# reazon-research/ReazonSpeech

Hardware: AMD Instinct MI355X
Metric: RTFx (audio-sec/wall-sec), FastConformer-RNNT 619M batch=256 (higher is better)
Workload: dtype bf16

## Files before the change

reazonspeech_amd/csrc/k_conformer.hip:

```cpp
#include <algorithm>

#include "rs_common.h"

extern "C" int rs_create(rs_ctx** out, int device, const rs_dims* dims) {
    if (!out || !dims) return RS_EINVAL;
    *out = nullptr;
    rs_ctx* ctx = new (std::nothrow) rs_ctx();
    rs_conformer* state = ctx ? new (std::nothrow) rs_conformer() : nullptr;
    if (!state) { delete ctx; return RS_EINVAL; }
    rs_conformer& cf = *state;
    ctx->family = RS_FAM_CONFORMER;
    ctx->state.reset(state);
    ctx->device = device;
    ctx->d = *dims;
    const rs_dims& d = ctx->d;
    int rc = RS_OK;
    if (d.n_heads <= 0 || d.d_model % d.n_heads || (d.d_model / d.n_heads != 128 && d.d_model / d.n_heads != 64))
        rc = rs_fail(ctx, RS_EINVAL, "head_dim must be 128 or 64 (d_model %d, heads %d)", d.d_model, d.n_heads);
    else if (d.d_model % 256 || d.ff_dim % 64) rc = rs_fail(ctx, RS_EINVAL, "d_model %% 256, ff_dim %% 64 required");
    else if (d.sub_stages < 2 || d.sub_stages > 4) rc = rs_fail(ctx, RS_EINVAL, "2..4 subsampling stages supported");
    else if (d.n_layers < 1) rc = rs_fail(ctx, RS_EINVAL, "n_layers");
    else if (d.pred_layers < 1 || d.pred_layers > 4) rc = rs_fail(ctx, RS_EINVAL, "pred_layers");
    else if ((unsigned)d.frontend_kind > 1u  || (unsigned)d.sub_kind > 1u || (unsigned)d.final_norm > 1u || (unsigned)d.joint_act > 1u)
        rc = rs_fail(ctx, RS_EINVAL, "model family switches must be 0 or 1");
// ... 295 lines not shown
        RS_TRY(gemm(ctxb, dm, L32.pw2_w, dm, x, dm, M, dm, RES, L.pw2_b, 1.0f, x));
        RS_TRY(rs_launch_layernorm(ctx, x, L.ln_ff2_g, L.ln_ff2_b, M, dm, d.ln_eps, nullptr, hn, s));
        RS_TRY(gemm(hn, dm, L32.ff2_w1, dm, big, ff, M, ff, RS_GEMM_BIAS | RS_GEMM_SILU, L.ff2_b1, 1.0f, nullptr));
        RS_TRY(gemm(big, ff, L32.ff2_w2, ff, x, dm, M, dm, RES, L.ff2_b2, 0.5f, x));
        RS_TRY(rs_launch_layernorm(ctx, x, L.ln_out_g, L.ln_out_b, M, dm, d.ln_eps, nullptr, x, s));
        for (size_t k = 0; k < cf.tap_ids.size(); ++k)
            if (cf.tap_ids[k] == i)
                RS_HIP(ctx, hipMemcpyAsync(cf.tap_layers + k * (size_t)M * dm, x, (size_t)M * dm * 4, hipMemcpyDeviceToDevice, s));
    }
    if (d.final_norm) RS_TRY(rs_launch_layernorm(ctx, x, cf.final_norm_g, cf.final_norm_b, M, dm, d.ln_eps, nullptr, x, s));
    if (enc_out) RS_HIP(ctx, hipMemcpyAsync(enc_out, x, (size_t)M * dm * 4, hipMemcpyDeviceToDevice, s));
    RS_TRY(gemm(x, dm, w.jenc_w, dm, joint_enc, d.joint_hidden, M, d.joint_hidden, RS_GEMM_BIAS, ctx->jenc_b, 1.0f, nullptr));
    if (d.ctc_vocab > 0 && (cf.ctc_probs || cf.ctc_blank)) {
        const int Vp = rs_ctc_pad(d.ctc_vocab);
        float* z = cf.ctc_probs ? cf.ctc_probs : pl.ctc;
        RS_TRY(gemm(x, dm, w.ctc_w, dm, z, Vp, M, Vp, RS_GEMM_BIAS, cf.ctc_b, 1.0f, nullptr));
        RS_TRY(rs_launch_ctc_softmax(ctx, z, M, d.ctc_vocab, Vp, d.blank_id, cf.ctc_blank, s));
    }
#undef RS_TRY
    return RS_OK;
}

}

size_t rs_conformer_workspace_bytes_impl(const rs_ctx* ctx, int B, int t_max) {
    rs_arena measure;
    plan_encoder(ctx, B, t_max > 0 ? t_max : 1, measure);
    size_t enc = measure.bytes() + ENC_SLACK;
    if (ctx->has_f32) {
        const size_t enc32 = encoder_f32_workspace_bytes(ctx, B, t_max > 0 ? t_max : 1);
        if (enc32 > enc) enc = enc32;
    }
    return enc;
}

int rs_conformer_encoder_forward_impl(rs_ctx* ctx, const float* feats, const int32_t* n_frames, int B, int t_max, float* enc_out, float* joint_enc,
                                      int32_t* enc_lens, void* workspace, size_t workspace_bytes, hipStream_t s) {
    if (ctx->precision_f32)
        return rs_encoder_forward_f32(ctx, feats, n_frames, B, t_max, enc_out, joint_enc, enc_lens, workspace, workspace_bytes, s);
    const rs_dims& d = ctx->d;
    const rs_conformer& cf = *rs_conformer_of(ctx);
    rs_arena arena(workspace);
    const EncPlan pl = plan_encoder(ctx, B, t_max, arena);
    if (workspace_bytes < arena.bytes() + ENC_SLACK)
        return rs_fail(ctx, RS_EWORKSPACE, "encoder: workspace %zu < %zu", workspace_bytes, arena.bytes() + ENC_SLACK);
    int32_t* const lens_stage = pl.lens;
    uint16_t *const sa = pl.sa, *const sb = pl.sb, *const hn = pl.hn, *const big = pl.big, *const ctxb = pl.ctxb, *const posp = pl.posp;
    float *const x = pl.x, *const ln_stats = pl.stats;
    const int C = d.sub_channels, dm = d.d_model, ff = d.ff_dim, S = d.sub_stages;
    const int Tp = pl.T[S], M = B * Tp;
    int rc;
#define RS_TRY(call) do { rc = (call); if (rc != RS_OK) return rc; } while (0)

    RS_TRY(rs_launch_enc_lens(ctx, n_frames, B, lens_stage, s));
    if (Tp <= 0) return rs_fail(ctx, RS_EINVAL, "encoder: %d feature frames are too few for the subsampling", t_max);
    if (d.sub_kind == 1) {
        uint16_t* const col = pl.col;
        const int T1 = pl.T[1], F1 = pl.F[1], T2 = pl.T[2], F2 = pl.F[2];
        for (int b0 = 0; b0 < B; b0 += pl.chunk) {
            const int bc = B - b0 < pl.chunk ? B - b0 : pl.chunk;
            RS_TRY(rs_launch_sub2d_conv0(ctx, feats, lens_stage, b0, bc, t_max, T1, F1, sa, s));
            const bool patches_in_place = col == nullptr;
            if (!patches_in_place) RS_TRY(rs_launch_im2col3x3s2(ctx, sa, bc, T1, F1, T2, F2, col, s));
            rs_gemm_args g{};
            if (patches_in_place) { g.A = sa; g.conv_C = C; g.conv_T1 = T1; g.conv_F1 = F1; g.conv_T2 = T2; g.conv_F2 = F2; }
            else g.A = col;
            g.lda = 9 * C; g.W = cf.sub_conv1_w; g.ldw = 9 * C; g.out = sb + (size_t)b0 * T2 * F2 * C; g.ldc = C;
            g.M = bc * T2 * F2; g.N = C; g.K = 9 * C;
            g.flags = RS_GEMM_BIAS | RS_GEMM_RELU | RS_GEMM_ROWMASK; g.bias = cf.sub_conv1_b; g.alpha = 1.0f;
            g.mask_lens = lens_stage + B + b0; g.mask_rows_per_step = F2; g.mask_steps = T2;
            RS_TRY(rs_launch_gemm(ctx, g, s));
        }
    } else
    RS_TRY(rs_launch_sub_conv0_dw1(ctx, feats, lens_stage, B, t_max, pl.T[2], pl.F[2], sa, s));
    for (int st = 2; st <= S && d.sub_kind == 0; ++st) {
        if (st > 2)
            RS_TRY(rs_launch_sub_dw(ctx, sb, cf.sub_dw_w[st - 2], cf.sub_dw_b[st - 2], lens_stage + (st - 1) * B, st, B,
                                    pl.T[st - 1], pl.F[st - 1], pl.T[st], pl.F[st], sa, s));
        rs_gemm_args g{};
        g.A = sa; g.lda = C; g.W = cf.sub_pw_w[st - 2]; g.ldw = C; g.out = sb; g.ldc = C;
        g.M = B * pl.T[st] * pl.F[st]; g.N = C; g.K = C;
        g.flags = RS_GEMM_BIAS | RS_GEMM_RELU | RS_GEMM_ROWMASK; g.bias = cf.sub_pw_b[st - 2]; g.alpha = 1.0f;
        g.mask_lens = lens_stage + (st - 1) * B; g.mask_rows_per_step = pl.F[st]; g.mask_steps = pl.T[st];
        RS_TRY(rs_launch_gemm(ctx, g, s));
    }
    {
        rs_gemm_args g{};
        const int K = C * pl.F[S];
        g.A = sb; g.lda = K; g.W = cf.sub_out_w; g.ldw = K; g.out = x; g.ldc = dm; g.M = M; g.N = dm; g.K = K;
        g.flags = RS_GEMM_BIAS | RS_GEMM_OUT_F32; g.bias = cf.sub_out_b;
        g.alpha = d.xscaling ? sqrtf((float)dm) : 1.0f;
        RS_TRY(rs_launch_gemm(ctx, g, s));
    }
    const int32_t* lens = lens_stage + (S - 1) * B;
    RS_HIP(ctx, hipMemcpyAsync(enc_lens, lens, (size_t)B * 4, hipMemcpyDeviceToDevice, s));
    if (cf.tap_sub) RS_HIP(ctx, hipMemcpyAsync(cf.tap_sub, x, (size_t)M * dm * 4, hipMemcpyDeviceToDevice, s));

    const int tcap = (int)((cf.pos_table_bytes / ((size_t)dm * 2) + 1) / 2);
    if (Tp > tcap) return rs_fail(ctx, RS_EINVAL, "encoder: T'=%d exceeds the registered pos.table capacity %d", Tp, tcap);
    const uint16_t* pos_slice = cf.pos_table + (size_t)(tcap - Tp) * dm;
    const int npos = 2 * Tp - 1;

    const rs_layer_w* res_ln = nullptr;
    auto gemm = [&](const uint16_t* A, int lda, const uint16_t* W, int K, void* out, int ldc, int Mr, int N, int flags,
                    const float* bias, float alpha, const float* res) -> int {
        rs_gemm_args g{};
        g.A = A; g.lda = lda; g.W = W; g.ldw = K; g.out = out; g.ldc = ldc; g.M = Mr; g.N = N; g.K = K;
        g.flags = flags; g.bias = bias; g.alpha = alpha; g.residual = res;
        if (res && res_ln) { g.res_ln_stats = ln_stats; g.res_ln_g = res_ln->ln_out_g; g.res_ln_b = res_ln->ln_out_b; res_ln = nullptr; }
        return rs_launch_gemm(ctx, g, s);
    };
    const int RES = RS_GEMM_BIAS | RS_GEMM_RESIDUAL | RS_GEMM_OUT_F32;
    const bool glu_fused = cf.fuse_glu != 0 && (dm % 32) == 0;

    for (int i = 0; i < d.n_layers; ++i) {
        const rs_layer_w& L = cf.layers[i];
        const bool last = i == d.n_layers - 1;
        if (i == 0) RS_TRY(rs_launch_layernorm(ctx, x, L.ln_ff1_g, L.ln_ff1_b, M, dm, d.ln_eps, hn, nullptr, s));
        RS_TRY(gemm(hn, dm, L.ff1_w1, dm, big, ff, M, ff, RS_GEMM_BIAS | RS_GEMM_SILU, L.ff1_b1, 1.0f, nullptr));
        RS_TRY(gemm(big, ff, L.ff1_w2, ff, x, dm, M, dm, RES, L.ff1_b2, 0.5f, x));
        RS_TRY(rs_launch_layernorm(ctx, x, L.ln_att_g, L.ln_att_b, M, dm, d.ln_eps, hn, nullptr, s));
        RS_TRY(gemm(hn, dm, L.qkv_w, dm, big, 3 * dm, M, 3 * dm, RS_GEMM_BIAS, L.qkv_b, 1.0f, nullptr));
        const uint16_t* pproj = posp;
        if (L.pos_proj) pproj = L.pos_proj + (size_t)(tcap - Tp) * dm;
        else RS_TRY(gemm(pos_slice, dm, L.pos_w, dm, posp, dm, npos, dm, 0, nullptr, 1.0f, nullptr));
        RS_TRY(rs_launch_attention(ctx, big, pproj, L.bias_u, L.bias_v, lens, B, Tp, ctxb, s));
        RS_TRY(gemm(ctxb, dm, L.out_w, dm, x, dm, M, dm, RES, L.out_b, 1.0f, x));
        RS_TRY(rs_launch_layernorm(ctx, x, L.ln_conv_g, L.ln_conv_b, M, dm, d.ln_eps, hn, nullptr, s));
        if (glu_fused) {
            RS_TRY(gemm(hn, dm, L.pw1_w, dm, big, dm, M, 2 * dm, RS_GEMM_BIAS | RS_GEMM_GLU, L.pw1_b, 1.0f, nullptr));
            RS_TRY(rs_launch_glu_dwconv(ctx, big, RS_GLU_APPLIED, L.dw_w, L.dw_b, lens, B, Tp, dm, d.conv_kernel, ctxb, s));
        } else {
            RS_TRY(gemm(hn, dm, L.pw1_w, dm, big, 2 * dm, M, 2 * dm, RS_GEMM_BIAS, L.pw1_b, 1.0f, nullptr));
            RS_TRY(rs_launch_glu_dwconv(ctx, big, RS_GLU_BLOCK32, L.dw_w, L.dw_b, lens, B, Tp, dm, d.conv_kernel, ctxb, s));
        }
        RS_TRY(gemm(ctxb, dm, L.pw2_w, dm, x, dm, M, dm, RES, L.pw2_b, 1.0f, x));
        RS_TRY(rs_launch_layernorm(ctx, x, L.ln_ff2_g, L.ln_ff2_b, M, dm, d.ln_eps, hn, nullptr, s));
        RS_TRY(gemm(hn, dm, L.ff2_w1, dm, big, ff, M, ff, RS_GEMM_BIAS | RS_GEMM_SILU, L.ff2_b1, 1.0f, nullptr));
        RS_TRY(gemm(big, ff, L.ff2_w2, ff, x, dm, M, dm, RES, L.ff2_b2, 0.5f, x));
        if (last && d.final_norm) {
            RS_TRY(rs_launch_layernorm(ctx, x, L.ln_out_g, L.ln_out_b, M, dm, d.ln_eps, nullptr, x, s));
        } else if (last) {
            bool want_f32 = enc_out != nullptr;
            for (size_t k = 0; k < cf.tap_ids.size(); ++k) want_f32 = want_f32 || cf.tap_ids[k] == i;
            RS_TRY(rs_launch_layernorm(ctx, x, L.ln_out_g, L.ln_out_b, M, dm, d.ln_eps, hn, want_f32 ? x : nullptr, s));
        } else {
            const rs_layer_w& Ln = cf.layers[i + 1];
            bool tapped = cf.defer_out_norm == 0;
            for (size_t k = 0; k < cf.tap_ids.size(); ++k) tapped = tapped || cf.tap_ids[k] == i;
            RS_TRY(rs_launch_layernorm2(ctx, x, L.ln_out_g, L.ln_out_b, Ln.ln_ff1_g, Ln.ln_ff1_b, M, dm, d.ln_eps,
                                        tapped ? x : nullptr, hn, tapped ? nullptr : ln_stats, s));
            if (!tapped) res_ln = &L;
        }
        for (size_t k = 0; k < cf.tap_ids.size(); ++k)
            if (cf.tap_ids[k] == i)
                RS_HIP(ctx, hipMemcpyAsync(cf.tap_layers + k * (size_t)M * dm, x, (size_t)M * dm * 4, hipMemcpyDeviceToDevice, s));
    }
    if (d.final_norm) RS_TRY(rs_launch_layernorm(ctx, x, cf.final_norm_g, cf.final_norm_b, M, dm, d.ln_eps, hn, enc_out ? x : nullptr, s));
    if (enc_out) RS_HIP(ctx, hipMemcpyAsync(enc_out, x, (size_t)M * dm * 4, hipMemcpyDeviceToDevice, s));
    RS_TRY(gemm(hn, dm, ctx->jenc_w, dm, joint_enc, d.joint_hidden, M, d.joint_hidden, RS_GEMM_BIAS | RS_GEMM_OUT_F32,
                ctx->jenc_b, 1.0f, nullptr));
    if (d.ctc_vocab > 0 && (cf.ctc_probs || cf.ctc_blank)) {
        float* z = cf.ctc_probs ? cf.ctc_probs : pl.ctc;
        const int Vp = rs_ctc_pad(d.ctc_vocab);
        RS_TRY(gemm(hn, dm, cf.ctc_w, dm, z, Vp, M, Vp, RS_GEMM_BIAS | RS_GEMM_OUT_F32, cf.ctc_b, 1.0f, nullptr));
        RS_TRY(rs_launch_ctc_softmax(ctx, z, M, d.ctc_vocab, Vp, d.blank_id, cf.ctc_blank, s));
    }
// ... 4 lines not shown
```

reazonspeech_amd/csrc/k_subsample.hip:

```cpp
#include "rs_common.h"

namespace {

__global__ void enc_lens_kernel(const int32_t* __restrict__ n_frames, int B, int stages, int sub_kind, int32_t* __restrict__ out) {
    const int b = blockIdx.x * blockDim.x + threadIdx.x;
    if (b >= B) return;
    int n = n_frames[b];
    for (int s = 0; s < stages; ++s) {
        n = n > 0 ? (sub_kind ? (n >= 3 ? (n - 3) / 2 + 1 : 0) : (n + 2 - 3) / 2 + 1) : 0;
        out[s * B + b] = n;
    }
}

__device__ __forceinline__ void put(uint16_t* p, float v) { *p = f32_to_bf16(v); }
__device__ __forceinline__ void put(float* p, float v) { *p = v; }

template <typename OT>
__global__ __launch_bounds__(256) void sub_conv0_dw1_kernel(
    const float* __restrict__ feats, const int32_t* __restrict__ lens_stage , int B, int t_max,
    int n_mels, int T2, int F1, int F2, int C, const float* __restrict__ w0 ,
    const float* __restrict__ b0, const float* __restrict__ wd , const float* __restrict__ bd,
    OT* __restrict__ out) {
    const int b = blockIdx.y, t2 = blockIdx.x, c = threadIdx.x;
    const int L1 = lens_stage[0 * B + b], L2 = lens_stage[1 * B + b];
// ... 292 lines not shown
        float wt[9][8], bs[8];
#pragma unroll
        for (int k = 0; k < 9; ++k) {
            const float4 w0 = reinterpret_cast<const float4*>(w + k * C + c)[0], w1 = reinterpret_cast<const float4*>(w + k * C + c)[1];
            wt[k][0] = w0.x; wt[k][1] = w0.y; wt[k][2] = w0.z; wt[k][3] = w0.w; wt[k][4] = w1.x; wt[k][5] = w1.y; wt[k][6] = w1.z; wt[k][7] = w1.w;
        }
        {
            const float4 b0 = reinterpret_cast<const float4*>(bias + c)[0], b1 = reinterpret_cast<const float4*>(bias + c)[1];
            bs[0] = b0.x; bs[1] = b0.y; bs[2] = b0.z; bs[3] = b0.w; bs[4] = b1.x; bs[5] = b1.y; bs[6] = b1.z; bs[7] = b1.w;
        }
        bool jok[3];
#pragma unroll
        for (int j = 0; j < 3; ++j) { const int fi = 2 * fo - 1 + j; jok[j] = fi >= 0 && fi < Fin; }
        const uint16_t* ibase = in + ((size_t)b * Tin * Fin) * C + c;
        auto load_row = [&](int ti, u16x8_t (&x)[3]) {
#pragma unroll
            for (int j = 0; j < 3; ++j) {
                if (jok[j]) x[j] = *reinterpret_cast<const u16x8_t*>(ibase + ((size_t)ti * Fin + (2 * fo - 1 + j)) * C);
                else
#pragma unroll
                    for (int e = 0; e < 8; ++e) x[j][e] = 0;
            }
        };
        u16x8_t top[3], mid[3], bot[3];
#pragma unroll
        for (int j = 0; j < 3; ++j)
#pragma unroll
            for (int e = 0; e < 8; ++e) { top[j][e] = 0; mid[j][e] = 0; bot[j][e] = 0; }
        bool top_ok = to_first > 0 && 2 * to_first - 1 < Tin;
        if (top_ok) load_row(2 * to_first - 1, top);
        u16x8_t mid_next[3], bot_next[3];
#pragma unroll
        for (int j = 0; j < 3; ++j) { mid_next[j] = mid[j]; bot_next[j] = bot[j]; }
        if (2 * to_first < Tin) load_row(2 * to_first, mid_next);
        if (2 * to_first + 1 < Tin) load_row(2 * to_first + 1, bot_next);
        for (int to = to_first; to < to_live; ++to) {
            const bool mid_ok = 2 * to < Tin, bot_ok = 2 * to + 1 < Tin;
#pragma unroll
            for (int j = 0; j < 3; ++j) { mid[j] = mid_next[j]; bot[j] = bot_next[j]; }
            if (to + 1 < to_live) {
                if (2 * to + 2 < Tin) load_row(2 * to + 2, mid_next);
                if (2 * to + 3 < Tin) load_row(2 * to + 3, bot_next);
            }
            float acc[8];
#pragma unroll
            for (int e = 0; e < 8; ++e) acc[e] = bs[e];
            if (top_ok) dw_taps(acc, wt, 0, top, jok);
            if (mid_ok) dw_taps(acc, wt, 1, mid, jok);
            if (bot_ok) dw_taps(acc, wt, 2, bot, jok);
            u16x8_t o;
#pragma unroll
            for (int e = 0; e < 8; ++e) o[e] = f32_to_bf16(acc[e]);
            *reinterpret_cast<u16x8_t*>(obase + ((size_t)to * Fout) * C) = o;
#pragma unroll
            for (int j = 0; j < 3; ++j) top[j] = bot[j];
            top_ok = bot_ok;
        }
    }
    u16x8_t z;
#pragma unroll
    for (int e = 0; e < 8; ++e) z[e] = 0;
    for (int to = max(to_first, to_live); to < to_end; ++to) *reinterpret_cast<u16x8_t*>(obase + ((size_t)to * Fout) * C) = z;
}

__global__ __launch_bounds__(256) void sub_dw_f32_kernel(const float* __restrict__ in, const float* __restrict__ w ,
                                                         const float* __restrict__ bias, const int32_t* __restrict__ lens_out,
                                                         int Tin, int Fin, int Tout, int Fout, int C, float* __restrict__ out) {
    const int c = threadIdx.x, fo = blockIdx.x, to = blockIdx.y, b = blockIdx.z;
    float* op = out + (((size_t)b * Tout + to) * Fout + fo) * C + c;
    if (to >= lens_out[b]) { *op = 0.0f; return; }
    float acc = bias[c];
#pragma unroll
    for (int i = 0; i < 3; ++i) {
        const int ti = 2 * to - 1 + i;
        if (ti < 0 || ti >= Tin) continue;
#pragma unroll
        for (int j = 0; j < 3; ++j) {
            const int fi = 2 * fo - 1 + j;
            if (fi < 0 || fi >= Fin) continue;
            acc = fmaf(w[(i * 3 + j) * C + c], in[(((size_t)b * Tin + ti) * Fin + fi) * C + c], acc);
        }
    }
    *op = acc;
}

}

int rs_launch_enc_lens(rs_ctx* ctx, const int32_t* n_frames, int B, int32_t* lens_out, hipStream_t s) {
    hipLaunchKernelGGL(enc_lens_kernel, dim3((B + 127) / 128), dim3(128), 0, s, n_frames, B, ctx->d.sub_stages, ctx->d.sub_kind, lens_out);
    RS_CHECK_LAUNCH(ctx, "enc_lens");
    return RS_OK;
}

constexpr int SUB_F2 = 20;
static bool conv0_run_form(int F2) { return F2 == SUB_F2 && !rs_knob(RS_KNOB_SUB_CONV0_OLD); }

int rs_launch_sub_conv0_dw1(rs_ctx* ctx, const float* feats, const int32_t* lens_stage, int B, int t_max, int T2,
                            int F2, uint16_t* out, hipStream_t s) {
    const rs_dims& d = ctx->d;
    const rs_conformer& cf = *rs_conformer_of(ctx);
    const int C = d.sub_channels;
    if (C > 256 || (C % 64)) return rs_fail(ctx, RS_EINVAL, "subsampling: channels %d unsupported (<=256, %%64)", C);
    const int F1 = (d.n_mels + 2 - 3) / 2 + 1;
    if (d.n_mels % 4 || 4 * F2 > d.n_mels || 2 * F2 < F1)
        return rs_fail(ctx, RS_EINVAL, "subsampling: n_mels=%d must be a multiple of 4 with 4*F2 <= n_mels", d.n_mels);
    const size_t lds = 0;
    const double flops = (double)B * T2 * F2 * C * 2.0 * (6 * 9 + 9);
    const double bytes = (double)B * t_max * d.n_mels * 4.0 + (double)B * T2 * F2 * C * 2.0;
    rs_prof_scope prof(ctx, RS_PROF_SUBSAMPLE, s, flops, bytes);
    if (conv0_run_form(F2))
        hipLaunchKernelGGL((sub_conv0_dw1_run_kernel<uint16_t, SUB_F2>), dim3((T2 + SUB_RUN - 1) / SUB_RUN, B), dim3(C / 2), lds, s, feats,
                           lens_stage, B, t_max, d.n_mels, T2, C, cf.sub_conv0_w, cf.sub_conv0_b, cf.sub_dw_w[0], cf.sub_dw_b[0], out);
    else
        hipLaunchKernelGGL(sub_conv0_dw1_kernel<uint16_t>, dim3(T2, B), dim3(C), lds, s, feats, lens_stage, B, t_max, d.n_mels, T2,
                       F1, F2, C, cf.sub_conv0_w, cf.sub_conv0_b, cf.sub_dw_w[0], cf.sub_dw_b[0], out);
    prof.end();
    RS_CHECK_LAUNCH(ctx, "sub_conv0_dw1");
    return RS_OK;
}

int rs_launch_sub_dw(rs_ctx* ctx, const uint16_t* in, const float* w, const float* b, const int32_t* lens_out,
                     int stage, int B, int t_in, int f_in, int t_out, int f_out, uint16_t* out, hipStream_t s) {
    (void)stage;
    const int C = ctx->d.sub_channels;
    const int cgs = C / 8;
    const int fpb = 256 / cgs;
    const dim3 grid((f_out + fpb - 1) / fpb, t_out, B), block(cgs * fpb);
    const double bytes = (double)B * C * 2.0 * ((double)t_in * f_in + (double)t_out * f_out);
    rs_prof_scope prof(ctx, RS_PROF_SUBSAMPLE, s, (double)B * t_out * f_out * C * 18.0, bytes);
    if (!rs_knob(RS_KNOB_SUB_DW_OLD) && cgs * f_out <= 512)
        hipLaunchKernelGGL(sub_dw_run_kernel, dim3((t_out + DW_RUN - 1) / DW_RUN, B), dim3(cgs * f_out), 0, s, in, w, b, lens_out, t_in,
                           f_in, t_out, f_out, C, out);
    else
        hipLaunchKernelGGL(sub_dw_kernel, grid, block, 0, s, in, w, b, lens_out, t_in, f_in, t_out, f_out, C, out);
    prof.end();
    RS_CHECK_LAUNCH(ctx, "sub_dw");
    return RS_OK;
}

int rs_launch_sub_conv0_dw1_f32(rs_ctx* ctx, const float* feats, const int32_t* lens_stage, int B, int t_max, int T2, int F2,
                                float* out, hipStream_t s) {
    const rs_dims& d = ctx->d;
    const rs_conformer& cf = *rs_conformer_of(ctx);
    const int C = d.sub_channels;
    if (C > 256 || (C % 64)) return rs_fail(ctx, RS_EINVAL, "subsampling: channels %d unsupported (<=256, %%64)", C);
    const int F1 = (d.n_mels + 2 - 3) / 2 + 1;
    if (d.n_mels % 4 || 4 * F2 > d.n_mels || 2 * F2 < F1)
        return rs_fail(ctx, RS_EINVAL, "subsampling: n_mels=%d must be a multiple of 4 with 4*F2 <= n_mels", d.n_mels);
    rs_prof_scope prof(ctx, RS_PROF_SUBSAMPLE, s, (double)B * T2 * F2 * C * 2.0 * (6 * 9 + 9),
                       (double)B * t_max * d.n_mels * 4.0 + (double)B * T2 * F2 * C * 4.0);
    if (conv0_run_form(F2))
        hipLaunchKernelGGL((sub_conv0_dw1_run_kernel<float, SUB_F2>), dim3((T2 + SUB_RUN - 1) / SUB_RUN, B), dim3(C / 2), 0, s, feats,
                           lens_stage, B, t_max, d.n_mels, T2, C, cf.sub_conv0_w, cf.sub_conv0_b, cf.sub_dw_w[0], cf.sub_dw_b[0], out);
    else
        hipLaunchKernelGGL(sub_conv0_dw1_kernel<float>, dim3(T2, B), dim3(C), 0, s, feats, lens_stage, B, t_max, d.n_mels, T2, F1, F2, C,
                       cf.sub_conv0_w, cf.sub_conv0_b, cf.sub_dw_w[0], cf.sub_dw_b[0], out);
    prof.end();
    RS_CHECK_LAUNCH(ctx, "sub_conv0_dw1_f32");
    return RS_OK;
}

int rs_launch_sub_dw_f32(rs_ctx* ctx, const float* in, const float* w, const float* b, const int32_t* lens_out, int B, int t_in,
                         int f_in, int t_out, int f_out, float* out, hipStream_t s) {
    const int C = ctx->d.sub_channels;
    rs_prof_scope prof(ctx, RS_PROF_SUBSAMPLE, s, (double)B * t_out * f_out * C * 18.0,
                       (double)B * C * 4.0 * ((double)t_in * f_in + (double)t_out * f_out));
    hipLaunchKernelGGL(sub_dw_f32_kernel, dim3(f_out, t_out, B), dim3(C), 0, s, in, w, b, lens_out, t_in, f_in, t_out, f_out, C, out);
    prof.end();
    RS_CHECK_LAUNCH(ctx, "sub_dw_f32");
    return RS_OK;
}
```

reazonspeech_amd/csrc/rs_common.h:

```cpp
#pragma once
#include <hip/hip_runtime.h>
#include <stdint.h>
#include <stdio.h>
#include <memory>
#include <string>
#include <unordered_map>
#include <vector>

#include "../../include/rs_asr.h"
#include "rs_arena.h"
#include "rs_family.h"
#include "rs_knobs.h"
#include "rs_tensors.h"

typedef __bf16 bf16x8_t __attribute__((ext_vector_type(8)));
typedef float f32x4_t __attribute__((ext_vector_type(4)));
typedef float f32x16_t __attribute__((ext_vector_type(16)));
typedef unsigned short u16x8_t __attribute__((ext_vector_type(8)));
typedef unsigned short u16x4_t __attribute__((ext_vector_type(4)));

__device__ __forceinline__ float bf16_to_f32(unsigned short v) {
    return __uint_as_float(((unsigned)v) << 16);
}
typedef __bf16 bf16x4_t __attribute__((ext_vector_type(4)));
// ... 124 lines not shown
    void* wfm_scratch = nullptr;
    size_t wfm_scratch_bytes = 0;
    int prof_mask = 0;
    rs_prof_slot prof[8];
    int32_t prof_tag[4] = {0, 0, 0, 0};
};

inline rs_conformer* rs_conformer_of(const rs_ctx* ctx) {
    return ctx && ctx->family == RS_FAM_CONFORMER ? static_cast<rs_conformer*>(ctx->state.get()) : nullptr;
}
rs_k2* rs_k2_of(const rs_ctx* ctx);
rs_avsr* rs_avsr_of(const rs_ctx* ctx);

int rs_ensure_dynamic_lds(rs_ctx* ctx, const void* func, int bytes);

int rs_fail(rs_ctx* ctx, int code, const char* fmt, ...);

inline int rs_guard(rs_ctx* ctx, rs_entry e) {
    char msg[512];
    const int rc = rs_family_guard(e, ctx != nullptr, ctx ? ctx->family : RS_FAM_CONFORMER, ctx && ctx->finalized, msg, sizeof msg);
    if (rc != RS_OK && ctx) ctx->err = msg;
    return rc;
}
inline bool rs_guard_query(const rs_ctx* ctx, rs_entry e) {
    return rs_family_guard(e, ctx != nullptr, ctx ? ctx->family : RS_FAM_CONFORMER, ctx && ctx->finalized, nullptr, 0) == RS_OK;
}
#define RS_GUARD(ctx, entry) do { if (const int _g = rs_guard((ctx), RS_ENTRY_##entry); _g != RS_OK) return _g; } while (0)
#define RS_GUARD_QUERY(ctx, entry, zero) do { if (!rs_guard_query((ctx), RS_ENTRY_##entry)) return zero; } while (0)

struct rs_weights : rs_tensor_reader {
    explicit rs_weights(const rs_ctx* ctx) : rs_tensor_reader(ctx->tensors) {}
    template <typename T>
    void get(const std::string& name, size_t elems, const T*& out) {
        const void* p = out;
        get_bytes(name, elems * sizeof(T), p);
        out = static_cast<const T*>(p);
    }
    int fail(rs_ctx* ctx) const { return rs_fail(ctx, rc, "%s", msg.c_str()); }
};
void rs_get_screened_joint(rs_ctx* ctx, rs_weights& r);
int rs_n_cus(rs_ctx* ctx);

#define RS_HIP(ctx, call)                                                              \
    do {                                                                               \
        hipError_t _e = (call);                                                        \
        if (_e != hipSuccess)                                                          \
            return rs_fail((ctx), RS_EHIP, "%s:%d %s -> %s", __FILE__, __LINE__, #call, \
                           hipGetErrorString(_e));                                     \
    } while (0)

#define RS_CHECK_LAUNCH(ctx, what)                                                            \
    do {                                                                                      \
        hipError_t _e = hipGetLastError();                                                    \
        if (_e != hipSuccess)                                                                 \
            return rs_fail((ctx), RS_EHIP, "launch %s failed: %s", (what), hipGetErrorString(_e)); \
    } while (0)

int rs_prof_class_index(int klass);
void rs_prof_begin(rs_ctx* ctx, int klass, hipStream_t s, double flops, double bytes);
void rs_prof_end(rs_ctx* ctx, int klass, hipStream_t s);
struct rs_prof_scope {
    rs_prof_scope(rs_ctx* ctx, int klass, hipStream_t s, double flops, double bytes) : ctx(ctx), klass(klass), s(s) { rs_prof_begin(ctx, klass, s, flops, bytes); }
    rs_prof_scope(const rs_prof_scope&) = delete;
    rs_prof_scope& operator=(const rs_prof_scope&) = delete;
    ~rs_prof_scope() { end(); }
    void end() { if (open) rs_prof_end(ctx, klass, s); open = false; }
private:
    rs_ctx* ctx; int klass; hipStream_t s; bool open = true;
};

struct rs_gemm_args {
    const uint16_t* A; int lda;
    const uint16_t* W; int ldw;
    void* out; int ldc;
    int M, N, K, flags;
    const float* bias; float alpha;
    const float* residual;
    const int32_t* mask_lens; int mask_rows_per_step; int mask_steps;
    const float* res_ln_stats; const float* res_ln_g; const float* res_ln_b;
    uint16_t* out_bf16; int ld_bf16;
    int conv_C, conv_T1, conv_F1, conv_T2, conv_F2;
};
int rs_launch_gemm(rs_ctx* ctx, const rs_gemm_args& a, hipStream_t s);
int rs_launch_layernorm(rs_ctx* ctx, const float* x, const float* g, const float* b, int M, int d, float eps,
                        uint16_t* out_bf16, float* out_f32, hipStream_t s);
int rs_launch_layernorm2(rs_ctx* ctx, const float* x, const float* g1, const float* b1, const float* g2, const float* b2,
                         int M, int d, float eps, float* out_f32, uint16_t* out_bf16, float* stats, hipStream_t s);
int rs_launch_attention(rs_ctx* ctx, const uint16_t* qkv, const uint16_t* pos, const float* bias_u,
                        const float* bias_v, const int32_t* lens, int B, int T, uint16_t* out, hipStream_t s);
int rs_launch_glu_dwconv(rs_ctx* ctx, const uint16_t* x, int layout, const float* w, const float* b, const int32_t* lens,
                         int B, int T, int d, int k, uint16_t* out, hipStream_t s);
int rs_launch_frontend(rs_ctx* ctx, const float* audio, const int32_t* lens, int B, int audio_stride,
                       int pad_left, int pad_right, int t_max, float* feats, int32_t* n_frames, float* raw,
                       hipStream_t s);
int rs_launch_sub_conv0_dw1(rs_ctx* ctx, const float* feats, const int32_t* lens_stage, int B, int t_max, int T2,
                            int F2, uint16_t* out, hipStream_t s);
int rs_launch_sub_dw(rs_ctx* ctx, const uint16_t* in, const float* w, const float* b, const int32_t* lens_out,
                     int stage, int B, int t_in, int f_in, int t_out, int f_out, uint16_t* out, hipStream_t s);
int rs_launch_gemm_f32(rs_ctx* ctx, const float* A, int lda, const float* W, int ldw, float* out, int ldc, int M, int N, int K,
                       int flags, const float* bias, float alpha, const float* residual, const int32_t* mask_lens,
                       int mask_rows_per_step, int mask_steps, hipStream_t s);
int rs_launch_conv3x3_f32(rs_ctx* ctx, const float* in, int n_img, int H, int Wd, int C, int OH, int OW, int stride, const float* W, int Cout,
                          const float* bn_scale, const float* bn_shift, const float* residual, const float* prelu, float* out, int one_by_one, hipStream_t s);
int rs_launch_gemm_f32_skinny(rs_ctx* ctx, const float* A, int lda, const float* W, int ldw, float* out, int ldc, int M, int N, int K, int flags,
                              const float* bias, const float* residual, hipStream_t s);
int rs_launch_attention_f32(rs_ctx* ctx, const float* qkv, const float* pos, const float* bias_u, const float* bias_v,
                            const int32_t* lens, int B, int T, float* out, hipStream_t s);
int rs_launch_glu_dwconv_f32(rs_ctx* ctx, const float* x, const float* w, const float* b, const int32_t* lens, int B, int T,
                             int d, int k, float* out, hipStream_t s);
int rs_launch_i8_range(rs_ctx* ctx, const float* A, int lda, const int32_t* lens, int group, int n_groups, int K, float* qp, hipStream_t s);
int rs_launch_gemm_i8q(rs_ctx* ctx, const float* A, int lda, int group, const float* qp, const int8_t* W, int ldw, const int32_t* colsum,
                       const float* wq, float* out, int ldc, int M, int N, int K, int flags, const float* bias, const float* residual, hipStream_t s);
int rs_launch_sub_conv0_dw1_f32(rs_ctx* ctx, const float* feats, const int32_t* lens_stage, int B, int t_max, int T2, int F2,
                                float* out, hipStream_t s);
int rs_launch_sub_dw_f32(rs_ctx* ctx, const float* in, const float* w, const float* b, const int32_t* lens_out, int B, int t_in,
                         int f_in, int t_out, int f_out, float* out, hipStream_t s);
int rs_launch_enc_lens(rs_ctx* ctx, const int32_t* n_frames, int B, int32_t* lens_out, hipStream_t s);
int rs_launch_sub2d_conv0(rs_ctx* ctx, const float* feats, const int32_t* lens1, int b0, int Bc, int t_max, int T1, int F1,
                          uint16_t* out, hipStream_t s);
int rs_launch_im2col3x3s2(rs_ctx* ctx, const uint16_t* in, int Bc, int T1, int F1, int T2, int F2, uint16_t* out, hipStream_t s);
int rs_launch_ctc_softmax(rs_ctx* ctx, float* logits, int M, int V, int ld, int blank, float* blank_out, hipStream_t s);
int rs_launch_sub2d_conv0_f32(rs_ctx* ctx, const float* feats, const int32_t* lens1, int b0, int Bc, int t_max, int T1, int F1,
                              float* out, hipStream_t s);
int rs_launch_im2col3x3s2_f32(rs_ctx* ctx, const float* in, int Bc, int T1, int F1, int T2, int F2, float* out, hipStream_t s);
static inline int rs_ctc_pad(int v) { return (v + 3) / 4 * 4; }
int rs_conformer_finalize_impl(rs_ctx* ctx);
size_t rs_conformer_workspace_bytes_impl(const rs_ctx* ctx, int B, int t_max);
int rs_conformer_encoder_forward_impl(rs_ctx* ctx, const float* feats, const int32_t* n_frames, int B, int t_max, float* enc_out, float* joint_enc,
                                      int32_t* enc_lens, void* workspace, size_t workspace_bytes, hipStream_t s);
int rs_avsr_finalize_impl(rs_ctx* ctx);
const rs_avsr_dims* rs_avsr_dims_of(const rs_ctx* ctx);
int rs_k2_finalize_impl(rs_ctx* ctx);
int rs_k2_unk_id(const rs_ctx* ctx);
size_t rs_k2_workspace_bytes_impl(const rs_ctx* ctx, int B, int t_max);
int rs_k2_enc_frames_impl(const rs_ctx* ctx, int n_feat);
int rs_k2_encoder_forward_impl(rs_ctx* ctx, const float* feats, const int32_t* n_frames, int B, int t_max, float* enc_out, float* joint_enc,
                               int32_t* enc_lens, void* workspace, size_t workspace_bytes, hipStream_t s);
int rs_launch_dwconv_act(rs_ctx* ctx, const uint16_t* x, const float* w, const float* b, const int32_t* lens, int B, int T, int d, int k,
                         int act, uint16_t* out, hipStream_t s);
static inline int rs_conv_len(int n, int sub_kind) { return sub_kind ? (n >= 3 ? (n - 3) / 2 + 1 : 0) : (n > 0 ? (n + 2 - 3) / 2 + 1 : 0); }
```

reazonspeech_amd/csrc/rs_knobs.h:

```cpp
#pragma once
#include <stdlib.h>
#include <string.h>

#include <atomic>
#include <mutex>

#include "../../include/rs_asr.h"

#define RS_KNOBS(X)                                                                                                                   \
    X(GEMM_TILE, "RS_GEMM_TILE", INT, 0, "forced GEMM tile height (256 / 192 / 128 / 64); 0 = by shape")                              \
    X(GEMM_GROUP_M, "RS_GEMM_GROUP_M", INT, 0, "row panels per XCD tile group; 0 = by shape")                                         \
    X(GEMM_PAIRS, "RS_GEMM_PAIRS", INT, 2, "2 = two tiles per workgroup, LDS ring carried over; 1 = ring restarted; 0 = one tile")    \
    X(GEMM_BREG, "RS_GEMM_BREG", INT, 0, "1 = 256- / 192-row launches keep the weight operand out of LDS (global -> VGPR)")           \
    X(ATTN_PERSIST, "RS_ATTN_PERSIST", INT, 0, "1 = full attention on resident workgroups that walk the items (n >= 2: on n)")        \
    X(ATTN_STREAM, "RS_ATTN_STREAM", INT, 0, "1 = the streaming attention form (+ 16 x mask: phases left out, for timing)")           \
    X(ATTN64, "RS_ATTN64", INT, 4, "head_dim 64: key blocks per chunk; 0 = the one-workgroup-per-CU geometry")                        \
    X(ATTN64_NW, "RS_ATTN64_NW", INT, 4, "head_dim 64: waves per workgroup (the second number of $RS_ATTN64)")                        \
    X(ATTN_F32_OLD, "RS_ATTN_F32_OLD", PRESENT, 0, "float32 attention: the first form (one wave per key sum)")                        \
    X(ATTN_F32_KEYS, "RS_ATTN_F32_KEYS", PRESENT, 0, "float32 attention: the second form (keys over lanes, no MFMA)")                 \
    X(GLU_GENERIC, "RS_GLU_GENERIC", INT, 0, "GLU + depthwise conv: 1 = the any-kernel-size path, 2 = the f32-tile kernel on the gated layout") \
    X(SUB_IM2COL, "RS_SUB_IM2COL", PRESENT, 0, "ESPnet subsampling: gather the 3 x 3 patches into a matrix first (sizes the workspace too)") \
    X(FUSE_GLU, "RS_FUSE_GLU", INT, 1, "context default: 0 = GLU in the depthwise kernel, not the pw1 GEMM epilogue")                 \
    X(DEFER_OUT_NORM, "RS_DEFER_OUT_NORM", INT, 1, "context default: 0 = every output norm stores its f32 rows")                      \
    X(DECODE_SCREEN, "RS_DECODE_SCREEN", INT, 1, "context default: 0 = exact evaluation of every joint column")                       \
    X(DECODE_NARROW, "RS_DECODE_NARROW", INT, 1, "context default: 0 = the wide-tile LSTM / projection kernels")                      \
    X(DECODE_NO_XCD, "RS_DECODE_NO_XCD", PRESENT, 0, "greedy decode: joint grids not padded to a multiple of 8 column tiles")         \
    X(DECODE_NO_LOOKAHEAD, "RS_DECODE_NO_LOOKAHEAD", PRESENT, 0, "greedy decode: one frame per utterance and step at every batch size") \
    X(VERIFY_WIDE, "RS_VERIFY_WIDE", INT, 0, "screened joint: 1 = a workgroup per row for V <= 3072 too")                             \
    X(DECODE_TRACE, "RS_DECODE_TRACE", PRESENT, 0, "greedy decode: print the step count of every call to stderr")                     \
    X(BEAM_SPEC, "RS_BEAM_SPEC", INT, 3, "beam search: evaluations asked for per iteration (1 .. 8; sizes the workspace too)")         \
    X(BEAM_TRACE, "RS_BEAM_TRACE", PRESENT, 0, "beam search: phase timing of the step kernel")                                        \
    X(BEAM_RECORD_LDS, "RS_BEAM_RECORD_LDS", PRESENT, 0, "beam search: the any-vocabulary record kernel on a small vocabulary")       \
    X(LOGMEL_OLD, "RS_LOGMEL_OLD", PRESENT, 0, "log-mel: the first form (16 frames per workgroup, filterbank read from global memory)") \
    X(SUB_CONV0_OLD, "RS_SUB_CONV0_OLD", PRESENT, 0, "conv0 + dw1: the first form (a workgroup per output row, every odd conv0 row twice)") \
    X(SUB_DW_OLD, "RS_SUB_DW_OLD", PRESENT, 0, "bf16 depthwise stage: the first form (a thread per output bin, every input row read by two rows)") \
    X(AVSR_POSCONV_OLD, "RS_AVSR_POSCONV_OLD", PRESENT, 0, "AV-HuBERT positional convolution: the VALU form")                         \
    X(K2_CONV1_OLD, "RS_K2_CONV1_OLD", PRESENT, 0, "Zipformer conv1: the VALU form (the one other channel counts run)")               \
    X(K2_ATTW_SWEEPS, "RS_K2_ATTW_SWEEPS", INT, 1, "Zipformer attention weights: 3 = the three-sweep kernel")                         \
    X(K2_CONV2_FUSED, "RS_K2_CONV2_FUSED", INT, 1, "default of option k2_conv2_fused: 0 = patch matrix + GEMM launch")                \
    X(K2_CNX_FUSED, "RS_K2_CNX_FUSED", INT, 1, "default of option k2_cnx_fused: 0 = the ConvNeXt pointwise pair as two GEMM launches")

enum rs_knob_id {
#define RS_KNOB_ENUM(id, env, kind, def, what) RS_KNOB_##id,
    RS_KNOBS(RS_KNOB_ENUM)
#undef RS_KNOB_ENUM
    RS_KNOB_COUNT
};
enum rs_knob_kind { RS_KNOB_PRESENT, RS_KNOB_INT };
struct rs_knob_row { const char* env; rs_knob_kind kind; int def; };
static const rs_knob_row rs_knob_rows[RS_KNOB_COUNT] = {
#define RS_KNOB_ROW(id, env, kind, def, what) {env, RS_KNOB_##kind, def},
    RS_KNOBS(RS_KNOB_ROW)
#undef RS_KNOB_ROW
};

struct rs_knob_table {
    std::atomic<int> value[RS_KNOB_COUNT];
    std::atomic<bool> given[RS_KNOB_COUNT];
    std::once_flag once;
};
inline rs_knob_table rs_knob_state;

inline void rs_knobs_read_env() {
    std::call_once(rs_knob_state.once, [] {
        rs_knob_table& t = rs_knob_state;
        for (int i = 0; i < RS_KNOB_COUNT; ++i) { t.value[i] = rs_knob_rows[i].def; t.given[i] = false; }
        for (int i = 0; i < RS_KNOB_COUNT; ++i) {
            const char* e = i == RS_KNOB_ATTN64_NW ? nullptr : getenv(rs_knob_rows[i].env);
            if (!e) continue;
            t.given[i] = true;
            t.value[i] = rs_knob_rows[i].kind == RS_KNOB_PRESENT ? 1 : atoi(e);
            if (i == RS_KNOB_ATTN64) {
                t.given[RS_KNOB_ATTN64_NW] = true;
                if (const char* c = strchr(e, ',')) t.value[RS_KNOB_ATTN64_NW] = atoi(c + 1);
            }
        }
    });
}

inline int rs_knob(rs_knob_id id) { rs_knobs_read_env(); return rs_knob_state.value[id].load(std::memory_order_relaxed); }
inline bool rs_knob_given(rs_knob_id id) { rs_knobs_read_env(); return rs_knob_state.given[id].load(std::memory_order_relaxed); }
inline void rs_knob_set(rs_knob_id id, int v) { rs_knobs_read_env(); rs_knob_state.value[id].store(v, std::memory_order_relaxed); }

inline int rs_knob_find(const char* env_name) {
    for (int i = 0; env_name && i < RS_KNOB_COUNT; ++i)
        if (!strcmp(env_name, rs_knob_rows[i].env)) return i;
    return -1;
}
inline int rs_knob_set_named(const char* env_name, int v) {
    const int i = rs_knob_find(env_name);
    if (i < 0) return RS_EINVAL;
    rs_knob_set((rs_knob_id)i, v);
    return RS_OK;
}
inline int rs_knob_get_named(const char* env_name, int* v) {
    const int i = rs_knob_find(env_name);
    if (i < 0 || !v) return RS_EINVAL;
    *v = rs_knob((rs_knob_id)i);
    return RS_OK;
}
```

Before: 47280.

## Add persistent streaming MFMA kernel for 256-channel subsampling pointwise convs

Routes the 256x256 pointwise convolutions of the subsampling stage through a dedicated persistent kernel instead of the generic GEMM. Each workgroup keeps the full weight matrix in registers and streams 128-row A tiles into swizzled LDS with double-buffered direct global-to-LDS loads. Bias, ReLU and the length row mask are fused, and output is staged through LDS for coalesced stores. Tiles are assigned per XCD in contiguous runs. This targets the memory-bound, low-K GEMM, at the cost of inline-asm complexity and a narrow applicability check, with a fallback to the old GEMM.

```diff
diff --git a/reazonspeech_amd/csrc/k_conformer.hip b/reazonspeech_amd/csrc/k_conformer.hip
--- a/reazonspeech_amd/csrc/k_conformer.hip
+++ b/reazonspeech_amd/csrc/k_conformer.hip
@@ -401,7 +401,7 @@
         g.M = B * pl.T[st] * pl.F[st]; g.N = C; g.K = C;
         g.flags = RS_GEMM_BIAS | RS_GEMM_RELU | RS_GEMM_ROWMASK; g.bias = cf.sub_pw_b[st - 2]; g.alpha = 1.0f;
         g.mask_lens = lens_stage + (st - 1) * B; g.mask_rows_per_step = pl.F[st]; g.mask_steps = pl.T[st];
-        RS_TRY(rs_launch_gemm(ctx, g, s));
+        RS_TRY(rs_launch_sub_pw(ctx, g, s));
     }
     {
         rs_gemm_args g{};
diff --git a/reazonspeech_amd/csrc/k_subsample.hip b/reazonspeech_amd/csrc/k_subsample.hip
--- a/reazonspeech_amd/csrc/k_subsample.hip
+++ b/reazonspeech_amd/csrc/k_subsample.hip
@@ -398,6 +398,125 @@
         }
     }
     *op = acc;
+}
+
+constexpr int SPW_C = 256, SPW_ROWB = SPW_C * 2;
+__device__ __forceinline__ void spw_glds16(unsigned voff, const void* sbase, unsigned lds_dst) {
+    asm volatile("s_mov_b32 m0, %2\n\ts_nop 0\n\tglobal_load_lds_dwordx4 %0, %1" :: "v"(voff), "s"(sbase), "s"(lds_dst) : "memory");
+}
+__device__ __forceinline__ int spw_scalar_load(const int32_t* p) {
+    int v;
+    asm volatile("s_load_dword %0, %1, 0x0\n\ts_waitcnt lgkmcnt(0)" : "=s"(v) : "s"(p) : "memory");
+    return v;
+}
+__device__ __forceinline__ int spw_piece(int c, int row) { return (c & 16) | ((c & 15) ^ (row & 15)); }
+
+constexpr int SPW_ROWS = 128, SPW_LDS = 2 * SPW_ROWS * SPW_ROWB;
+__global__ __launch_bounds__(512) void sub_pw_stream_kernel(const uint16_t* __restrict__ A, const uint16_t* __restrict__ W,
+                                                            const float* __restrict__ bias, const int32_t* __restrict__ mask_lens,
+                                                            int mask_F, int mask_FT, uint16_t* __restrict__ out, int rows) {
+    constexpr int ROWS = SPW_ROWS, TILE = ROWS * SPW_ROWB, MT = ROWS / 16, RPW = ROWS / 8, NQ = ROWS / 16;
+    extern __shared__ __attribute__((aligned(16))) char spw_smem[];
+    const int tid = threadIdx.x, lane = tid & 63, li = lane & 15, kq = lane >> 4;
+    const int wave = __builtin_amdgcn_readfirstlane(tid >> 6);
+    const unsigned lds0 = (unsigned)(size_t)(__attribute__((address_space(3))) char*)spw_smem;
+    const int n_tiles = (rows + ROWS - 1) / ROWS;
+    const int xcd = blockIdx.x & 7, per = gridDim.x >> 3;
+    const int q8 = n_tiles >> 3, r8 = n_tiles & 7;
+    const int run0 = xcd * q8 + (xcd < r8 ? xcd : r8), run1 = run0 + q8 + (xcd < r8 ? 1 : 0);
+    bf16x8_t wf[2][8];
+#pragma unroll
+    for (int t = 0; t < 2; ++t)
+#pragma unroll
+        for (int ks = 0; ks < 8; ++ks)
+            wf[t][ks] = *reinterpret_cast<const bf16x8_t*>(W + (size_t)(32 * wave + 16 * t + li) * SPW_C + 32 * ks + 8 * kq);
+    float4 b4[2];
+#pragma unroll
+    for (int t = 0; t < 2; ++t) b4[t] = *reinterpret_cast<const float4*>(bias + 32 * wave + 16 * t + 4 * kq);
+    auto issue_tile = [&](int tile, int buf) {
+        const long long gr0 = (long long)tile * ROWS;
+#pragma unroll
+        for (int jj = 0; jj < NQ; ++jj) {
+            const int q = wave + 8 * jj;
+            const int r = 2 * q + (lane >> 5), pc = lane & 31;
+            const long long left = rows - 1 - gr0;
+            const int rr = r < left ? r : (int)left;
+            const unsigned voff = (unsigned)(rr * SPW_ROWB + (spw_piece(pc, r) << 4));
+            spw_glds16(voff, reinterpret_cast<const char*>(A) + gr0 * SPW_ROWB, lds0 + buf * TILE + q * 1024);
+        }
+    };
+    int tile = run0 + (int)(blockIdx.x >> 3);
+    if (tile < run1) issue_tile(tile, 0);
+    int buf = 0;
+    bool first = true;
+    for (; tile < run1; tile += per, buf ^= 1) {
+        if (first) asm volatile("s_waitcnt vmcnt(0)" ::: "memory");
+        else asm volatile("s_waitcnt vmcnt(%0)" :: "n"(NQ) : "memory");
+        first = false;
+        __builtin_amdgcn_s_barrier();
+        asm volatile("" ::: "memory");
+        if (tile + per < run1) issue_tile(tile + per, buf ^ 1);
+        unsigned long long keep;
+        {
+            long long m = (long long)tile * ROWS + wave * RPW + (lane < RPW ? lane : RPW - 1);
+            m = m < rows ? m : rows - 1;
+            const int b = (int)((unsigned)m / (unsigned)mask_FT);
+            const int rem = (int)m - b * mask_FT;
+            const int b_lo = __builtin_amdgcn_readfirstlane(b), b_hi = __builtin_amdgcn_readlane(b, RPW - 1);
+            int len = 0;
+            for (int bb = b_lo; bb <= b_hi; ++bb) {
+                const int l = spw_scalar_load(mask_lens + bb);
+                len = b == bb ? l : len;
+            }
+            keep = __ballot((long long)rem < (long long)len * mask_F);
+        }
+        const char* As = spw_smem + buf * TILE;
+        u16x4_t ov[MT][2];
+#pragma unroll
+        for (int mt = 0; mt < MT; ++mt) {
+            const int row = 16 * mt + li;
+            f32x4_t acc[2] = {{0.f, 0.f, 0.f, 0.f}, {0.f, 0.f, 0.f, 0.f}};
+#pragma unroll
+            for (int ks = 0; ks < 8; ++ks) {
+                const bf16x8_t af = *reinterpret_cast<const bf16x8_t*>(As + row * SPW_ROWB + (spw_piece(4 * ks + kq, row) << 4));
+#pragma unroll
+                for (int t = 0; t < 2; ++t) acc[t] = __builtin_amdgcn_mfma_f32_16x16x32_bf16(wf[t][ks], af, acc[t], 0, 0, 0);
+            }
+#pragma unroll
+            for (int t = 0; t < 2; ++t)
+                ov[mt][t] = pack_bf16x4(fmaxf(acc[t][0] + b4[t].x, 0.f), fmaxf(acc[t][1] + b4[t].y, 0.f), fmaxf(acc[t][2] + b4[t].z, 0.f),
+                                        fmaxf(acc[t][3] + b4[t].w, 0.f));
+        }
+        asm volatile("s_waitcnt lgkmcnt(0)" ::: "memory");
+        __builtin_amdgcn_s_barrier();
+        asm volatile("" ::: "memory");
+        char* Os = spw_smem + buf * TILE;
+#pragma unroll
+        for (int mt = 0; mt < MT; ++mt) {
+            const int row = 16 * mt + li;
+#pragma unroll
+            for (int t = 0; t < 2; ++t) {
+                const int c = 4 * wave + 2 * t + (kq >> 1);
+                *reinterpret_cast<u16x4_t*>(Os + row * SPW_ROWB + (spw_piece(c, row) << 4) + 8 * (kq & 1)) = ov[mt][t];
+            }
+        }
+        asm volatile("s_waitcnt lgkmcnt(0)" ::: "memory");
+        __builtin_amdgcn_s_barrier();
+        asm volatile("" ::: "memory");
+        uint4 ot[NQ];
+#pragma unroll
+        for (int ps = 0; ps < NQ; ++ps) {
+            const int row = RPW * wave + 2 * ps + (lane >> 5), pc = lane & 31;
+            ot[ps] = *reinterpret_cast<const uint4*>(Os + row * SPW_ROWB + (spw_piece(pc, row) << 4));
+        }
+#pragma unroll
+        for (int ps = 0; ps < NQ; ++ps) {
+            const int rl = 2 * ps + (lane >> 5), pc = lane & 31;
+            const uint4 v = ((keep >> rl) & 1) ? ot[ps] : make_uint4(0u, 0u, 0u, 0u);
+            const long long gr = (long long)tile * ROWS + RPW * wave + rl;
+            if (gr < rows) *reinterpret_cast<uint4*>(out + gr * SPW_C + 8 * pc) = v;
+        }
+    }
 }
 
 }
@@ -454,6 +573,39 @@
     return RS_OK;
 }
 
+int rs_launch_sub_pw(rs_ctx* ctx, const rs_gemm_args& g, hipStream_t s) {
+    const auto aligned16 = [](const void* p) { return p && !((uintptr_t)p & 15); };
+    const bool streams = !rs_knob(RS_KNOB_SUB_PW_OLD) && g.N == SPW_C && g.K == SPW_C && g.lda == SPW_C && g.ldw == SPW_C && g.ldc == SPW_C &&
+                         g.flags == (RS_GEMM_BIAS | RS_GEMM_RELU | RS_GEMM_ROWMASK) && g.alpha == 1.0f && !g.conv_C && g.M > 0 &&
+                         g.M <= INT32_MAX - 256 && aligned16(g.A) && aligned16(g.W) && aligned16(g.out) && aligned16(g.bias) && g.mask_lens &&
+                         g.mask_rows_per_step > 0 && g.mask_steps > 0 && (long long)g.mask_rows_per_step * g.mask_steps <= INT32_MAX;
+    if (!streams) return rs_launch_gemm(ctx, g, s);
+    const int n_tiles = (g.M + SPW_ROWS - 1) / SPW_ROWS;
+    int grid = rs_n_cus(ctx) / 8 * 8;
+    if (grid < 8) grid = 8;
+    if ((n_tiles + 7) / 8 * 8 < grid) grid = (n_tiles + 7) / 8 * 8;
+    if (int rc = rs_ensure_dynamic_lds(ctx, (const void*)sub_pw_stream_kernel, SPW_LDS); rc != RS_OK) return rc;
+    ctx->prof_tag[0] = g.M; ctx->prof_tag[1] = g.N; ctx->prof_tag[2] = g.K; ctx->prof_tag[3] = g.flags;
+    rs_prof_scope prof(ctx, RS_PROF_GEMM, s, 2.0 * g.M * (double)g.N * g.K, 2.0 * ((double)g.M * g.K + (double)g.N * g.K) + 2.0 * g.M * g.N);
+    const int FT = g.mask_rows_per_step * g.mask_steps;
+    hipLaunchKernelGGL(sub_pw_stream_kernel, dim3(grid), dim3(512), SPW_LDS, s, g.A, g.W, g.bias, g.mask_lens, g.mask_rows_per_step, FT,
+                       reinterpret_cast<uint16_t*>(g.out), g.M);
+    prof.end();
+    RS_CHECK_LAUNCH(ctx, "sub_pw_stream");
+    return RS_OK;
+}
+
+extern "C" int rs_debug_sub_pw(rs_ctx* ctx, const uint16_t* A, const uint16_t* W, const float* bias, const int32_t* lens, int M, int C,
+                               int rows_per_step, int steps, uint16_t* out, void* stream) {
+    if (!ctx) return RS_EINVAL;
+    if (!A || !W || !bias || !lens || !out) return rs_fail(ctx, RS_EINVAL, "sub_pw: null pointer");
+    rs_gemm_args g{};
+    g.A = A; g.lda = C; g.W = W; g.ldw = C; g.out = out; g.ldc = C; g.M = M; g.N = C; g.K = C;
+    g.flags = RS_GEMM_BIAS | RS_GEMM_RELU | RS_GEMM_ROWMASK; g.bias = bias; g.alpha = 1.0f;
+    g.mask_lens = lens; g.mask_rows_per_step = rows_per_step; g.mask_steps = steps;
+    return rs_launch_sub_pw(ctx, g, (hipStream_t)stream);
+}
+
 int rs_launch_sub_conv0_dw1_f32(rs_ctx* ctx, const float* feats, const int32_t* lens_stage, int B, int t_max, int T2, int F2,
                                 float* out, hipStream_t s) {
     const rs_dims& d = ctx->d;
diff --git a/reazonspeech_amd/csrc/rs_common.h b/reazonspeech_amd/csrc/rs_common.h
--- a/reazonspeech_amd/csrc/rs_common.h
+++ b/reazonspeech_amd/csrc/rs_common.h
@@ -230,6 +230,7 @@
     int conv_C, conv_T1, conv_F1, conv_T2, conv_F2;
 };
 int rs_launch_gemm(rs_ctx* ctx, const rs_gemm_args& a, hipStream_t s);
+int rs_launch_sub_pw(rs_ctx* ctx, const rs_gemm_args& a, hipStream_t s);
 int rs_launch_layernorm(rs_ctx* ctx, const float* x, const float* g, const float* b, int M, int d, float eps,
                         uint16_t* out_bf16, float* out_f32, hipStream_t s);
 int rs_launch_layernorm2(rs_ctx* ctx, const float* x, const float* g1, const float* b1, const float* g2, const float* b2,
diff --git a/reazonspeech_amd/csrc/rs_knobs.h b/reazonspeech_amd/csrc/rs_knobs.h
--- a/reazonspeech_amd/csrc/rs_knobs.h
+++ b/reazonspeech_amd/csrc/rs_knobs.h
@@ -34,6 +34,7 @@
     X(LOGMEL_OLD, "RS_LOGMEL_OLD", PRESENT, 0, "log-mel: the first form (16 frames per workgroup, filterbank read from global memory)") \
     X(SUB_CONV0_OLD, "RS_SUB_CONV0_OLD", PRESENT, 0, "conv0 + dw1: the first form (a workgroup per output row, every odd conv0 row twice)") \
     X(SUB_DW_OLD, "RS_SUB_DW_OLD", PRESENT, 0, "bf16 depthwise stage: the first form (a thread per output bin, every input row read by two rows)") \
+    X(SUB_PW_OLD, "RS_SUB_PW_OLD", PRESENT, 0, "256-channel pointwise convs of the subsampling: the GEMM launch, not the streaming kernel") \
     X(AVSR_POSCONV_OLD, "RS_AVSR_POSCONV_OLD", PRESENT, 0, "AV-HuBERT positional convolution: the VALU form")                         \
     X(K2_CONV1_OLD, "RS_K2_CONV1_OLD", PRESENT, 0, "Zipformer conv1: the VALU form (the one other channel counts run)")               \
     X(K2_ATTW_SWEEPS, "RS_K2_ATTW_SWEEPS", INT, 1, "Zipformer attention weights: 3 = the three-sweep kernel")                         \
```

Result: no change. 47410 (median of 6 runs) (+0.3%).
